# abdo-eldesokey/RAFT-NCUP

Hardware: AMD Instinct MI355X
Metric: train_image_pairs_per_sec (higher is better)
Workload: dtype bf16; 1 GPU; model=raft_nc_dbl, global_batch=3, refinement_iters=12, parallelism=dp1

## Files before the change

### csrc/bindings.cpp

```cpp

#include <torch/extension.h>

#include <vector>

#include <ATen/cuda/CUDAContext.h>
#include <c10/cuda/CUDAGuard.h>
#include <hip/hip_runtime.h>

void flowhip_bgemm_nt_launch(const void* A, const void* B, void* C,
                             float alpha, int batch, int M, int N, int K,
                             int out_bf16, hipStream_t stream);
void flowhip_corr_lookup_fwd_launch(const void* const* levels, const int* Hs,
                                    const int* Ws, const float* coords,
                                    void* out, int BP, int P,
                                    int L, int radius, int cl, int ldc,
                                    int is_bf16, hipStream_t stream);
void flowhip_corr_lookup_bwd_launch(const void* gout, const float* coords,
                                    void* const* glevels, const int* Hs,
                                    const int* Ws, int BP, int P,
                                    int L, int radius, int cl,
                                    int is_bf16, int acc,
                                    hipStream_t stream);
void flowhip_convex_up_fwd_launch(const float* flow, const float* mask,
                                  float* out, int N, int H, int W, int factor,
                                  hipStream_t stream);
void flowhip_convex_up_bwd_launch(const float* gout, const float* flow,
                                  const float* mask, float* gflow,
                                  float* gmask, int N, int H, int W,
                                  int factor, hipStream_t stream);
void flowhip_nconv_fwd_launch(const float* data, const float* conf,
                              const float* weight, const float* bias,
                              float* out, float* cout, int N, int Ci, int Co,
                              int H, int W, int K, hipStream_t stream);
void flowhip_nconv_bwd_data_launch(const float* dnomin, const float* ddenom,
                                   const float* data, const float* conf,
                                   const float* weight, float* ddata,
                                   float* dconf, int N, int Ci, int Co, int H,
                                   int W, int K, hipStream_t stream);
void flowhip_nconv_wrw_launch(const float* dnomin, const float* ddenom,
                              const float* data, const float* conf,
                              float* dweight, int N, int Ci, int Co, int H,
                              int W, int K, hipStream_t stream);
int flowhip_nconv_tiled_nblocks(int N, int H, int W, int Ci);
bool flowhip_nconv_fwd_tiled_launch(const float* data, const float* conf,
                                    const float* weight, const float* bias,
                                    float* out, float* cout, int N, int Ci,
                                    int Co, int H, int W, int K,
                                    hipStream_t stream);
bool flowhip_nconv_bwd_data_tiled_launch(
    const float* dnomin, const float* ddenom, const float* data,
    const float* conf, const float* weight, float* ddata, float* dconf, int N,
    int Ci, int Co, int H, int W, int K, hipStream_t stream);
bool flowhip_nconv_wrw_tiled_launch(const float* dnomin, const float* ddenom,
                                    const float* data, const float* conf,
                                    float* partials, float* dweight, int N,
                                    int Ci, int Co, int H, int W, int K,
                                    hipStream_t stream);
int flowhip_instnorm_partial_rows(int N, int C, long P);
void flowhip_conv_gemm_pack_launch(const float* w, void* wpk, long total,
                                   int O, int I, int KH, int KW, int cpad,
                                   int flip, hipStream_t stream);
void flowhip_transpose_cast_launch(const void* in, void* out, int B, int M,
                                   int N, int in_bf16, hipStream_t stream);
void flowhip_conf_pool_fwd_launch(const float* data, const float* conf,
                                  float* data_ds, float* conf_ds,
                                  unsigned char* code, long total, int H,
                                  int W, int OH, int OW, hipStream_t stream);
void flowhip_conf_pool_bwd_launch(const float* gdata_ds,
                                  const float* gconf_ds,
                                  const unsigned char* code, float* gdata,
                                  float* gconf, long total_in, int H, int W,
                                  int OH, int OW, hipStream_t stream);
void flowhip_conv_gemm_fwd_launch(const void* x, const void* x2,
                                  const void* wpk, const float* bias,
                                  void* out, void* out2, const void* zpage,
                                  long Mtot, int HH, int WW, int srcH,
                                  int srcW, int sH, int sW, int ld_x,
                                  int ld_x2, int C1, int Cin, int Cout,
                                  int cpad, int KH, int KW, int padH,
                                  int padW, int osplit, int act, int smode,
                                  hipStream_t stream);
void flowhip_conv_gemm_wrw_launch(const void* dy, const void* x,
                                  const void* x2, float* partials, float* dw,
                                  float* dbias,
                                  const void* zpage, long Mtot, int HH,
                                  int WW, int srcH, int srcW, int sH, int sW,
                                  int ld_x, int ld_x2, int C1,
                                  int Cin, int Cout, int cpad, int KH,
                                  int KW, int padH, int padW, int nchunk,
                                  hipStream_t stream);
void flowhip_instnorm_cl_fwd_launch(const void* x, void* y, float* mean,
                                    float* rstd, float* partials, int N,
                                    int C, long P, float eps, int is_bf16,
                                    hipStream_t stream);
void flowhip_instnorm_cl_bwd_launch(const void* x, const void* dy,
                                    const float* mean, const float* rstd,
                                    float* gmean, float* gxmean,
                                    float* partials, void* dx, int N, int C,
                                    long P, int is_bf16, hipStream_t stream);
void flowhip_zero_inject_fwd_launch(const float* inp, float* out, long total,
                                    int ih, int iw, int oh, int ow, int sH,
                                    int sW, hipStream_t stream);
void flowhip_zero_inject_bwd_launch(const float* gout, float* dinp,
                                    long total, int ih, int iw, int oh,
                                    int ow, int sH, int sW,
                                    hipStream_t stream);
void flowhip_gru_gate1_fwd_launch(const void* zr, const void* h, void* z,
                                  void* rh, long total, int C, long P,
                                  int is_bf16, int cl, hipStream_t stream);
void flowhip_gru_gate1_bwd_launch(const void* dz, const void* drh,
                                  const void* zr, const void* h, void* dzr,
                                  void* dh, long total, int C, long P,
                                  int is_bf16, int cl, hipStream_t stream);
void flowhip_gru_gate2_fwd_launch(const void* qp, const void* z,
                                  const void* h, void* hnew, long total,
                                  int is_bf16, hipStream_t stream);
void flowhip_gru_gate2_bwd_launch(const void* dhnew, const void* qp,
                                  const void* z, const void* h, void* dqp,
                                  void* dz, void* dh, long total, int is_bf16,
                                  hipStream_t stream);
void flowhip_seq_loss_fwd_launch(const float* const* preds, int n,
                                 const float* gt, const float* valid,
                                 float* partials, float* out, long npix,
                                 long plane, float max_flow, float gamma,
                                 long numel_full, hipStream_t stream);
void flowhip_seq_loss_bwd_launch(const float* const* preds, float* const* dst,
                                 int n, const float* gt, const float* valid,
                                 const float* gloss, long npix, long plane,
                                 float max_flow, float gamma, long numel_full,
                                 hipStream_t stream);
void flowhip_nconv_bwd_prep_launch(const float* gout, const float* gcout,
                                   const float* out, const float* cout,
                                   const float* wsum, const float* bias,
                                   float* dnomin, float* ddenom, long total,
                                   long plane, int Co, float eps,
                                   hipStream_t stream);
bool flowhip_col_sum2_launch(const void* g, const void* x, float* out,
                             long M, int C, int nchunk,
                             hipStream_t stream);
void flowhip_frozen_bn_apply_launch(const void* x, void* y, const float* s,
                                    const float* t, long M, int C,
                                    hipStream_t stream);
void flowhip_plane_dot_sum_launch(const float* x, const float* y, float* out,
                                  long P, int B, int C, hipStream_t stream);
bool flowhip_col_sum_launch(const void* dy, float* out,
                            long M, int C, int nchunk, hipStream_t stream);
void flowhip_up2x_cat_fwd_launch(const float* low, const float* skip,
                                 float* out, long total, int C1, int C2,
                                 int H, int W, hipStream_t stream);
void flowhip_area_up2x_fwd_launch(const float* in, float* out, long total,
                                  int H, int W, hipStream_t stream);
void flowhip_area_up2x_bwd_launch(const float* gout, float* gin,
                                  long total_in, int H, int W,
                                  hipStream_t stream);
bool flowhip_packernel_fwd_launch(const float* f, float* k, int B, int C,
                                  int H, int W, int K, int dil, int norm,
                                  hipStream_t stream);
bool flowhip_packernel_bwd_launch(const float* f, const float* k,
                                  const float* dk, float* df, int B, int C,
                                  int H, int W, int K, int dil, int norm,
                                  hipStream_t stream);
bool flowhip_pacconv_fwd_launch(const float* x, const float* kr,
                                const float* w, const float* bias, float* out,
                                int B, int Ci, int Co, int H, int W, int OH,
                                int OW, int pH, int pW, int K, int dil,
                                int shared, hipStream_t stream);
bool flowhip_pacconv_bwd_launch(const float* dy, const float* x,
                                const float* kr, const float* w, float* dx,
                                float* dk, float* partials, float* dw,
                                int nchunk, int B, int Ci, int Co, int H,
                                int W, int OH, int OW, int pH, int pW, int K,
                                int dil, int shared, hipStream_t stream);
void flowhip_pacpool_fwd_launch(const float* x, const float* kr, float* out,
// ... 670 lines not shown
  return wpk;
}

std::vector<torch::Tensor> conv_gemm_fwd2(
    torch::Tensor x, c10::optional<torch::Tensor> x2, torch::Tensor wpk,
    c10::optional<torch::Tensor> bias, int64_t Cout, int64_t KH, int64_t KW,
    int64_t osplit, int64_t act, int64_t sH, int64_t sW, int64_t smode,
    int64_t outH, int64_t outW) {
  int ld_x, ld_x2 = 0;
  cg_check_x(x, ld_x);
  TORCH_CHECK(wpk.is_cuda() && wpk.is_contiguous() &&
              wpk.scalar_type() == torch::kBFloat16 && wpk.dim() == 3);
  const int N = x.size(0), C1 = x.size(1), H = x.size(2), W = x.size(3);
  int Cin = C1;
  const void* x2p = nullptr;
  if (x2.has_value()) {
    int l2;
    cg_check_x(x2.value(), l2);
    TORCH_CHECK(x2->size(0) == N && x2->size(2) == H && x2->size(3) == W);
    TORCH_CHECK(C1 % 64 == 0, "conv_gemm cat2: first input must be a "
                "multiple of 64 channels");
    ld_x2 = l2;
    Cin = C1 + (int)x2->size(1);
    x2p = x2->data_ptr();
  }
  const int cpad = wpk.size(2);
  TORCH_CHECK(wpk.size(0) == KH * KW && wpk.size(1) == Cout);
  TORCH_CHECK(smode >= 0 && smode <= 2 && sH >= 1 && sW >= 1);
  int OH = H, OW = W;
  if (smode == 1) {
    OH = (int)((H + 2 * (KH / 2) - KH) / sH + 1);
    OW = (int)((W + 2 * (KW / 2) - KW) / sW + 1);
  } else if (smode == 2) {
    TORCH_CHECK(outH > 0 && outW > 0, "conv_gemm smode=2 needs outH/outW");
    OH = (int)outH; OW = (int)outW;
  }
  const long Mtot = (long)N * OH * OW;
  const float* bptr = nullptr;
  if (bias.has_value()) {
    TORCH_CHECK(bias->is_contiguous() &&
                bias->scalar_type() == torch::kFloat32 &&
                bias->numel() == Cout);
    bptr = bias->data_ptr<float>();
  }
  const c10::cuda::CUDAGuard guard(x.device());
  hipStream_t stream = at::cuda::getCurrentCUDAStream().stream();
  if (osplit <= 0 || osplit >= Cout) {
    auto out = torch::empty({(long)N, Cout, (long)OH, (long)OW}, x.options(),
                            torch::MemoryFormat::ChannelsLast);
    flowhip_conv_gemm_fwd_launch(x.data_ptr(), x2p, wpk.data_ptr(), bptr,
                                 out.data_ptr(), nullptr, cg_zero_page(),
                                 Mtot, OH, OW, H, W, (int)sH, (int)sW, ld_x,
                                 ld_x2, C1, Cin, (int)Cout,
                                 cpad, (int)KH, (int)KW, (int)KH / 2,
                                 (int)KW / 2, (int)Cout, (int)act,
                                 (int)smode, stream);
    return {out};
  }
  TORCH_CHECK(smode == 0, "conv_gemm: osplit only with smode 0");
  auto out = torch::empty({(long)N, osplit, (long)H, (long)W}, x.options(),
                          torch::MemoryFormat::ChannelsLast);
  auto out2 = torch::empty({(long)N, Cout - osplit, (long)H, (long)W},
                           x.options(), torch::MemoryFormat::ChannelsLast);
  flowhip_conv_gemm_fwd_launch(x.data_ptr(), x2p, wpk.data_ptr(), bptr,
                               out.data_ptr(), out2.data_ptr(),
                               cg_zero_page(), Mtot, H, W, H, W, 1, 1, ld_x,
                               ld_x2, C1,
                               Cin, (int)Cout, cpad, (int)KH, (int)KW,
                               (int)KH / 2, (int)KW / 2, (int)osplit,
                               (int)act, 0, stream);
  return {out, out2};
}

torch::Tensor conv_gemm_fwd(torch::Tensor x, torch::Tensor wpk,
                            c10::optional<torch::Tensor> bias, int64_t Cout,
                            int64_t KH, int64_t KW, int64_t act) {
  return conv_gemm_fwd2(x, c10::nullopt, wpk, bias, Cout, KH, KW, 0,
                        act, 1, 1, 0, 0, 0)[0];
}

std::vector<torch::Tensor> conv_gemm_wrw(torch::Tensor dy, torch::Tensor x,
                                         c10::optional<torch::Tensor> x2,
                                         int64_t KH, int64_t KW, int64_t sH,
                                         int64_t sW, bool want_bias) {
  int ld_x, ld_x2 = 0;
  cg_check_x(x, ld_x);
  TORCH_CHECK(dy.is_cuda() && dy.scalar_type() == torch::kBFloat16 &&
              dy.stride(1) == 1 && dy.stride(3) == dy.size(1),
              "conv_gemm_wrw: dy must be channels-last contiguous");
  const int N = x.size(0), C1 = x.size(1), H = x.size(2), W = x.size(3);
  const int OH = dy.size(2), OW = dy.size(3);
  TORCH_CHECK(dy.size(0) == N);
  int Cin = C1;
  const void* x2p = nullptr;
  if (x2.has_value()) {
    int l2;
    cg_check_x(x2.value(), l2);
    ld_x2 = l2;
    Cin = C1 + (int)x2->size(1);
    x2p = x2->data_ptr();
  }
  const int Cout = dy.size(1);
  const long Mtot = (long)N * OH * OW;
  const int cpad = (int)((Cin + 63) / 64) * 64;
  const int tiles_o = (Cout + 63) / 64;
  const int base_tiles = tiles_o * ((cpad + 63) / 64) * (int)(KH * KW);
  int nchunk = (512 + base_tiles - 1) / base_tiles;
  if (nchunk < 1) nchunk = 1;
  if (nchunk > 64) nchunk = 64;
  const long mtiles = (Mtot + 63) / 64;
  if (nchunk > mtiles) nchunk = (int)mtiles;
  auto partials = torch::empty(
      {(long)nchunk * KH * KW * tiles_o * 64 * cpad +
       (want_bias ? (long)nchunk * tiles_o * 64 : 0)},
      x.options().dtype(torch::kFloat32));
  auto dw = torch::empty({(long)Cout, (long)Cin, KH, KW},
                         x.options().dtype(torch::kFloat32));
  torch::Tensor dbias;
  if (want_bias)
    dbias = torch::empty({(long)Cout}, x.options().dtype(torch::kFloat32));
  const c10::cuda::CUDAGuard guard(x.device());
  hipStream_t stream = at::cuda::getCurrentCUDAStream().stream();
  flowhip_conv_gemm_wrw_launch(dy.data_ptr(), x.data_ptr(), x2p,
                               partials.data_ptr<float>(),
                               dw.data_ptr<float>(),
                               want_bias ? dbias.data_ptr<float>() : nullptr,
                               cg_zero_page(), Mtot,
                               OH, OW, H, W, (int)sH, (int)sW,
                               ld_x, ld_x2, C1, Cin, Cout, cpad, (int)KH,
                               (int)KW, (int)KH / 2, (int)KW / 2, nchunk,
                               stream);
  return {dw, dbias};
}

torch::Tensor col_sum_bf16(torch::Tensor dy) {
  TORCH_CHECK(dy.is_cuda() && dy.dim() == 4 &&
              dy.scalar_type() == torch::kBFloat16 && dy.stride(1) == 1 &&
              dy.stride(3) == dy.size(1));
  const int C = dy.size(1);
  const long M = dy.numel() / C;
  const int nchunk = (int)((M + 255) / 256);
  auto out = torch::zeros({(long)C}, dy.options().dtype(torch::kFloat32));
  const c10::cuda::CUDAGuard guard(dy.device());
  hipStream_t stream = at::cuda::getCurrentCUDAStream().stream();
  bool ok = flowhip_col_sum_launch(dy.data_ptr(),
                                   out.data_ptr<float>(), M, C, nchunk,
                                   stream);
  TORCH_CHECK(ok, "col_sum_bf16: C must be a multiple of 8");
  return out;
}

torch::Tensor plane_sum_nchw(torch::Tensor x, c10::optional<torch::Tensor> y) {
  TORCH_CHECK(x.is_cuda() && x.dim() == 4 && x.is_contiguous() &&
              x.scalar_type() == torch::kFloat32);
  const float* yp = nullptr;
  if (y.has_value()) {
    TORCH_CHECK(y->sizes() == x.sizes() && y->is_contiguous() &&
                y->scalar_type() == torch::kFloat32);
    yp = y->data_ptr<float>();
  }
  const int B = x.size(0), C = x.size(1);
  const long P = (long)x.size(2) * x.size(3);
  auto out = torch::zeros({(long)C}, x.options());
  const c10::cuda::CUDAGuard guard(x.device());
  hipStream_t stream = at::cuda::getCurrentCUDAStream().stream();
  flowhip_plane_dot_sum_launch(x.data_ptr<float>(), yp,
                               out.data_ptr<float>(), P, B, C, stream);
  return out;
}

torch::Tensor frozen_bn_apply(torch::Tensor x, torch::Tensor s,
                              c10::optional<torch::Tensor> t) {
  TORCH_CHECK(x.is_cuda() && x.dim() == 4 &&
              x.scalar_type() == torch::kBFloat16 && x.stride(1) == 1 &&
              x.stride(3) == x.size(1) && x.size(1) % 8 == 0);
  TORCH_CHECK(s.is_contiguous() && s.scalar_type() == torch::kFloat32 &&
              s.numel() == x.size(1));
  const float* tp = nullptr;
  if (t.has_value()) {
    TORCH_CHECK(t->is_contiguous() && t->scalar_type() == torch::kFloat32 &&
                t->numel() == x.size(1));
    tp = t->data_ptr<float>();
  }
  auto y = torch::empty_like(x);
  const c10::cuda::CUDAGuard guard(x.device());
  hipStream_t stream = at::cuda::getCurrentCUDAStream().stream();
  flowhip_frozen_bn_apply_launch(x.data_ptr(), y.data_ptr(),
                                 s.data_ptr<float>(), tp,
                                 x.numel() / x.size(1), (int)x.size(1),
                                 stream);
  return y;
}

torch::Tensor col_sum2_bf16(torch::Tensor g, torch::Tensor x) {
  TORCH_CHECK(g.is_cuda() && g.dim() == 4 &&
              g.scalar_type() == torch::kBFloat16 && g.stride(1) == 1 &&
              g.stride(3) == g.size(1));
  TORCH_CHECK(x.sizes() == g.sizes() && x.strides() == g.strides() &&
              x.scalar_type() == torch::kBFloat16);
  const int C = g.size(1);
  const long M = g.numel() / C;
  const int nchunk = (int)((M + 255) / 256);
  auto out = torch::zeros({2, (long)C}, g.options().dtype(torch::kFloat32));
  const c10::cuda::CUDAGuard guard(g.device());
  hipStream_t stream = at::cuda::getCurrentCUDAStream().stream();
  bool ok = flowhip_col_sum2_launch(g.data_ptr(), x.data_ptr(),
                                    out.data_ptr<float>(), M, C, nchunk,
                                    stream);
  TORCH_CHECK(ok, "col_sum2_bf16: C must be a multiple of 8");
  return out;
}

torch::Tensor up2x_cat_fwd(torch::Tensor low, torch::Tensor skip) {
  TORCH_CHECK(low.is_cuda() && low.is_contiguous() &&
// ... 148 lines not shown
                                       int64_t sH, int64_t sW, int64_t pH,
                                       int64_t pW, int64_t dil) {
  const int B = x.size(0), C = x.size(1), H = x.size(2), W = x.size(3);
  const int KCH = kr.size(1), OH = kr.size(3), OW = kr.size(4);
  auto dx = torch::zeros_like(x);
  auto dk = torch::empty_like(kr);
  const c10::cuda::CUDAGuard guard(x.device());
  hipStream_t stream = at::cuda::getCurrentCUDAStream().stream();
  flowhip_pacpool_bwd_launch(dy.contiguous().data_ptr<float>(),
                             x.data_ptr<float>(), kr.data_ptr<float>(),
                             dx.data_ptr<float>(), dk.data_ptr<float>(), B,
                             C, KCH, H, W, OH, OW, (int)K, (int)sH, (int)sW,
                             (int)pH, (int)pW, (int)dil, stream);
  return {dx, dk};
}

}

PYBIND11_MODULE(TORCH_EXTENSION_NAME, m) {
  m.doc() = "flowhip gfx950 HIP kernels";
  m.def("bgemm_nt", &bgemm_nt,
        "C[b] = alpha * A[b] (M,K) @ B[b] (N,K)^T, bf16 in / fp32|bf16 out",
        py::arg("a"), py::arg("b"), py::arg("alpha"),
        py::arg("out_bf16") = false);
  m.def("corr_lookup_fwd", &corr_lookup_fwd,
        "fused multi-level correlation window lookup (fp32/bf16 levels)");
  m.def("corr_lookup_bwd", &corr_lookup_bwd,
        "backward of corr_lookup_fwd (pyramid grads; accumulates into "
        "`prev` when the pyramid is iteration-chained)",
        py::arg("gout"), py::arg("coords"), py::arg("radius"),
        py::arg("level_shapes"), py::arg("channels_last"),
        py::arg("levels_bf16") = false,
        py::arg("prev") = py::none());
  m.def("corr_pyramid_fits", &corr_pyramid_fits,
        "does the fused pyramid-build kernel support this map size/dtype");
  m.def("packernel_fwd", &packernel_fwd, "PAC gaussian adapting kernel");
  m.def("packernel_bwd", &packernel_bwd, "backward of packernel_fwd");
  m.def("pacconv_fwd", &pacconv_fwd, "pixel-adaptive convolution forward");
  m.def("pacconv_bwd", &pacconv_bwd, "pixel-adaptive conv backward (dx,dk,dw)");
  m.def("pacpool_fwd", &pacpool_fwd, "pixel-adaptive pooling forward");
  m.def("pacpool_bwd", &pacpool_bwd,
        "pixel-adaptive pooling backward (dx via atomic scatter, dk)");
  m.def("corr_pyramid_fwd", &corr_pyramid_fwd,
        "fused avg-pool pyramid build (levels 1..n-1)");
  m.def("corr_pyramid_bwd", &corr_pyramid_bwd,
        "fused pyramid backward combine -> dcorr");
  m.def("convex_up_fwd", &convex_up_fwd, "fused convex-combination upsample");
  m.def("convex_up_bwd", &convex_up_bwd, "backward of convex_up_fwd");
  m.def("nconv_fwd", &nconv_fwd,
        "fused normalized convolution forward (out, cout)");
  m.def("plane_sum_nchw", &plane_sum_nchw,
        "out[c] = sum_{b,h,w} x (or x*y), NCHW fp32",
        py::arg("x"), py::arg("y") = py::none());
  m.def("frozen_bn_apply", &frozen_bn_apply,
        "y = bf16(fp32(x)*s + t) per channel, channels-last");
  m.def("col_sum2_bf16", &col_sum2_bf16,
        "(sum_m g, sum_m g*x) per channel in one pass (frozen-BN backward)");
  m.def("col_sum_bf16", &col_sum_bf16,
        "(N,C,H,W) channels-last bf16 -> (C) fp32 bias-grad column sum");
  m.def("up2x_cat_fwd", &up2x_cat_fwd,
        "fused nearest-2x upsample + channel concat");
  m.def("area_up2x_fwd", &area_up2x_fwd, "exact-2x area upsample");
  m.def("area_up2x_bwd", &area_up2x_bwd, "backward of area_up2x");
  m.def("conf_pool_fwd", &conf_pool_fwd,
        "confidence-based 2x pooling forward (data_ds, conf_ds, argmax code)");
  m.def("conf_pool_bwd", &conf_pool_bwd, "backward of conf_pool");
  m.def("transpose_cast_bf16", &transpose_cast_bf16,
        "(B,M,N) fp32 -> (B,N,M) bf16 tiled transpose");
  m.def("conv_gemm_pack", &conv_gemm_pack,
        "one-kernel conv weight packing (fwd or flipped-bwd layout)");
  m.def("conv_gemm_fwd", &conv_gemm_fwd,
        "implicit-GEMM NHWC bf16 conv forward (also bwd-data with flipped "
        "packed weights)");
  m.def("conv_gemm_fwd2", &conv_gemm_fwd2,
        "conv forward over a virtually-concatenated pair of inputs and/or "
        "with a split output (bwd-data of a cat input); smode 1 = strided "
        "direct conv, smode 2 = strided transposed conv (bwd-data)",
        py::arg("x"), py::arg("x2"), py::arg("wpk"), py::arg("bias"),
        py::arg("Cout"), py::arg("KH"), py::arg("KW"), py::arg("osplit"),
        py::arg("act"), py::arg("sH") = 1, py::arg("sW") = 1,
        py::arg("smode") = 0, py::arg("outH") = 0, py::arg("outW") = 0);
  m.def("conv_gemm_wrw", &conv_gemm_wrw,
        "implicit-GEMM conv weight gradient (split-M + reduce); returns "
        "[dw, dbias] — dbias undefined unless want_bias",
        py::arg("dy"), py::arg("x"), py::arg("x2"), py::arg("KH"),
        py::arg("KW"), py::arg("sH") = 1, py::arg("sW") = 1,
        py::arg("want_bias") = false);
  m.def("instnorm_cl_fwd", &instnorm_cl_fwd,
        "channels-last InstanceNorm2d forward (y, mean, rstd)");
  m.def("instnorm_cl_bwd", &instnorm_cl_bwd,
        "channels-last InstanceNorm2d backward");
  m.def("zero_inject_fwd", &zero_inject_fwd, "sparse injection scatter");
  m.def("zero_inject_bwd", &zero_inject_bwd, "backward gather of inject");
  m.def("gru_gate1_fwd", &gru_gate1_fwd, "fused GRU z/r gates + r*h");
  m.def("gru_gate1_bwd", &gru_gate1_bwd, "backward of gru_gate1");
  m.def("gru_gate2_fwd", &gru_gate2_fwd, "fused GRU tanh + lerp update");
  m.def("gru_gate2_bwd", &gru_gate2_bwd, "backward of gru_gate2");
  m.def("seq_loss_fwd", &seq_loss_fwd,
        "fused sequence loss forward -> [loss, epe, 1px, 3px, 5px]");
  m.def("seq_loss_bwd", &seq_loss_bwd,
        "fused sequence loss backward -> per-prediction grads");
  m.def("nconv_bwd_prep", &nconv_bwd_prep,
        "fused elementwise preamble of nconv backward (dnomin, ddenom)");
  m.def("nconv_bwd", &nconv_bwd,
        "fused normalized convolution backward (ddata, dconf, dweight)");
}
```

### csrc/conv_gemm.hip

```cpp

#include "common.h"

#define CG_BM 64
#define CG_BN 64
#define CG_BK 64
#define CG_THREADS 256

__device__ __forceinline__ unsigned cg_swz(unsigned row, unsigned slot) {
  return slot ^ ((row >> 1) & 7u);
}

template <int BM, int THREADS>
__device__ __forceinline__ void cg_coords(
    int wave, int lane, long m0, long Mtot, int HH, int WW,
    long* pn, int* pyy, int* pxx) {
  constexpr int PPT = BM * 8 / THREADS;
#pragma unroll
  for (int j = 0; j < PPT; ++j) {
    const int piece = wave * 64 + THREADS * j + lane;
    long m = m0 + (piece >> 3);
    if (m >= Mtot) m = Mtot - 1;
    pxx[j] = (int)(m % WW);
    pyy[j] = (int)((m / WW) % HH);
    pn[j] = m / ((long)WW * HH);
  }
}

template <int BM, int THREADS, int SMODE>
__device__ __forceinline__ void cg_stage_a(
    const __bf16* __restrict__ x, const __bf16* __restrict__ x2,
    const __bf16* __restrict__ zpage,
    char* lds_buf, int wave, int lane, const long* pn, const int* pyy,
    const int* pxx, int srcH, int srcW, int sH, int sW, int ld_x, int ld_x2,
    int C1, int Cin, int dy, int dx, int c0) {
  constexpr int PPT = BM * 8 / THREADS;
#pragma unroll
  for (int j = 0; j < PPT; ++j) {
    const int piece0 = wave * 64 + THREADS * j;
    const int piece = piece0 + lane;
    const int row = piece >> 3;
    const int slot = piece & 7;
    const int sslot = cg_swz(row, slot);
    const int xx = pxx[j];
    const int yy = pyy[j];
    const long n = pn[j];
    int sy, sx;
    bool ok;
    if (SMODE == 0) {
      sy = yy + dy; sx = xx + dx;
      ok = sy >= 0 && sy < srcH && sx >= 0 && sx < srcW;
    } else if (SMODE == 1) {
      sy = yy * sH + dy; sx = xx * sW + dx;
      ok = sy >= 0 && sy < srcH && sx >= 0 && sx < srcW;
    } else {
      const int ty = yy + dy, tx = xx + dx;
      sy = ty / sH; sx = tx / sW;
      ok = ty >= 0 && tx >= 0 && ty % sH == 0 && tx % sW == 0 &&
           sy < srcH && sx < srcW;
    }
    const int c = c0 + sslot * 8;
    const __bf16* src = zpage;
    if (ok && c < Cin) {
      if (x2 == nullptr || c < C1)
        src = x + (((long)n * srcH + sy) * srcW + sx) * ld_x + c;
      else
        src = x2 + (((long)n * srcH + sy) * srcW + sx) * ld_x2 + (c - C1);
    }
    __builtin_amdgcn_global_load_lds(
        (const __attribute__((address_space(1))) void*)src,
        (__attribute__((address_space(3))) void*)(lds_buf + piece0 * 16),
        16, 0, 0);
  }
}

template <int THREADS>
__device__ __forceinline__ void cg_stage_b(const __bf16* __restrict__ wsec,
                                           char* lds_buf, int wave, int lane,
                                           int n0, int Cout, int cpad,
                                           int c0) {
  constexpr int PPT = CG_BN * 8 / THREADS;
#pragma unroll
  for (int j = 0; j < PPT; ++j) {
    const int piece0 = wave * 64 + THREADS * j;
    if (piece0 >= CG_BN * 8) break;
// ... 384 lines not shown
    }
  const long total = (long)Cout * Cin * KYX;
  for (long idx = (long)blockIdx.x * CG_THREADS + threadIdx.x; idx < total;
       idx += (long)gridDim.x * CG_THREADS) {
    long t = idx;
    const int kyx = (int)(t % KYX); t /= KYX;
    const int c = (int)(t % Cin); t /= Cin;
    const int o = (int)t;
    float s = 0.f;
    for (int ch = 0; ch < nchunk; ++ch)
      s += partials[((((long)ch * KYX + kyx) * orows) + o) * cpad + c];
    dw[((long)o * Cin + c) * KYX + kyx] = s;
  }
}


template <int BM>
static void cg_fwd_dispatch(const __bf16* x, const __bf16* x2,
                            const __bf16* wpk, const float* bias, __bf16* out,
                            __bf16* out2, const __bf16* zpage, long Mtot,
                            int HH, int WW, int srcH, int srcW, int sH,
                            int sW, int ld_x, int ld_x2, int C1, int Cin,
                            int Cout, int cpad, int KH, int KW, int offH,
                            int offW, int osplit, int act, int smode,
                            hipStream_t stream) {
  const int tiles_m = (int)((Mtot + BM - 1) / BM);
  const int tiles_n = fh_cdiv(Cout, CG_BN);
  dim3 grid(tiles_m * tiles_n), block(BM == 64 ? 256 : 512);
#define CG_LAUNCH(A, S)                                                      \
  hipLaunchKernelGGL((conv_gemm_fwd_kernel<A, BM, S>), grid, block, 0,       \
                     stream, x, x2, wpk, bias, out, out2, zpage, Mtot, HH,   \
                     WW, srcH, srcW, sH, sW, ld_x, ld_x2, C1, Cin, Cout,     \
                     cpad, KH, KW, offH, offW, osplit, tiles_m)
  if (smode == 0) { if (act == 1) CG_LAUNCH(1, 0); else CG_LAUNCH(0, 0); }
  else if (smode == 1) { if (act == 1) CG_LAUNCH(1, 1); else CG_LAUNCH(0, 1); }
  else { if (act == 1) CG_LAUNCH(1, 2); else CG_LAUNCH(0, 2); }
#undef CG_LAUNCH
}

bool flowhip_conv_halo_fwd_launch(const void* x, const void* x2,
                                  const void* wpk, const float* bias,
                                  void* out, const void* zpage, int N,
                                  int H, int W, int ld_x, int ld_x2, int C1,
                                  int Cin, int Cout, int cpad, int ldo,
                                  int KH, int KW, int act,
                                  hipStream_t stream);

void flowhip_conv_gemm_fwd_launch(const void* x, const void* x2,
                                  const void* wpk, const float* bias,
                                  void* out, void* out2, const void* zpage,
                                  long Mtot, int HH, int WW, int srcH,
                                  int srcW, int sH, int sW, int ld_x,
                                  int ld_x2, int C1, int Cin, int Cout,
                                  int cpad, int KH, int KW, int padH,
                                  int padW, int osplit, int act, int smode,
                                  hipStream_t stream) {
  if (smode == 0 && out2 == nullptr && padH == KH / 2 && padW == KW / 2 &&
      ((KH == 3 && KW == 3) || (KH == 1 && KW == 5) ||
       (KH == 5 && KW == 1))) {
    const int N = (int)(Mtot / ((long)HH * WW));
    if (flowhip_conv_halo_fwd_launch(x, x2, wpk, bias, out, zpage, N, HH,
                                     WW, ld_x, ld_x2, C1, Cin, Cout, cpad,
                                     Cout, KH, KW, act, stream))
      return;
  }
  const int offH = smode == 2 ? padH - KH + 1 : -padH;
  const int offW = smode == 2 ? padW - KW + 1 : -padW;
  const long t128 = ((Mtot + 127) / 128) * fh_cdiv(Cout, CG_BN);
  if (t128 >= 320)
    cg_fwd_dispatch<128>((const __bf16*)x, (const __bf16*)x2,
                         (const __bf16*)wpk, bias, (__bf16*)out,
                         (__bf16*)out2, (const __bf16*)zpage, Mtot, HH, WW,
                         srcH, srcW, sH, sW, ld_x, ld_x2, C1, Cin, Cout,
                         cpad, KH, KW, offH, offW, osplit, act, smode,
                         stream);
  else
    cg_fwd_dispatch<64>((const __bf16*)x, (const __bf16*)x2,
                        (const __bf16*)wpk, bias, (__bf16*)out, (__bf16*)out2,
                        (const __bf16*)zpage, Mtot, HH, WW, srcH, srcW, sH,
                        sW, ld_x, ld_x2, C1, Cin, Cout, cpad, KH, KW, offH,
                        offW, osplit, act, smode, stream);
}

void flowhip_conv_gemm_wrw_launch(const void* dy, const void* x,
                                  const void* x2, float* partials, float* dw,
                                  float* dbias, const void* zpage, long Mtot,
                                  int HH,
                                  int WW, int srcH, int srcW, int sH, int sW,
                                  int ld_x, int ld_x2, int C1, int Cin,
                                  int Cout, int cpad, int KH, int KW,
                                  int padH, int padW, int nchunk,
                                  hipStream_t stream) {
  const int tiles_o = fh_cdiv(Cout, 64);
  const int tiles_c = fh_cdiv(cpad, 64);
  float* biasp = dbias
      ? partials + (long)nchunk * KH * KW * tiles_o * 64 * cpad
      : nullptr;
  dim3 block(CG_THREADS);
  dim3 grid(tiles_o * tiles_c, KH * KW, nchunk);
  hipLaunchKernelGGL(conv_gemm_wrw_kernel, grid, block, 0, stream,
                     (const __bf16*)dy, (const __bf16*)x,
                     (const __bf16*)x2, partials, biasp,
                     (const __bf16*)zpage,
                     Mtot, HH, WW, srcH, srcW, sH, sW, ld_x, ld_x2, C1,
                     Cin, Cout, cpad, KH, KW, padH, padW, tiles_o, tiles_c,
                     nchunk);
  const long total = (long)Cout * Cin * KH * KW;
  long rblocks = (total + CG_THREADS - 1) / CG_THREADS;
  if (rblocks > 4096) rblocks = 4096;
  hipLaunchKernelGGL(conv_gemm_wrw_reduce_kernel, dim3((int)rblocks), block,
                     0, stream, partials, dw, biasp, dbias, nchunk, KH * KW,
                     tiles_o * 64, cpad, Cout, Cin);
}

__global__ __launch_bounds__(256) void conv_gemm_pack_kernel(
    const float* __restrict__ w,
    __bf16* __restrict__ wpk,
    long total, int O, int I, int KH, int KW, int cpad, int flip) {
  const int KYX = KH * KW;
  for (long idx = (long)blockIdx.x * 256 + threadIdx.x; idx < total;
       idx += (long)gridDim.x * 256) {
    long t = idx;
    const int c = t % cpad; t /= cpad;
    const int r = t % (flip ? I : O); t /= (flip ? I : O);
    const int kyx = (int)t;
    float v = 0.f;
    if (!flip) {
      if (c < I) v = w[(((long)r * I + c) * KYX) + kyx];
    } else {
      const int ky = kyx / KW, kx = kyx - (kyx / KW) * KW;
      const int fk = (KH - 1 - ky) * KW + (KW - 1 - kx);
      if (c < O) v = w[(((long)c * I + r) * KYX) + fk];
    }
    wpk[idx] = (__bf16)v;
  }
}

void flowhip_conv_gemm_pack_launch(const float* w, void* wpk, long total,
                                   int O, int I, int KH, int KW, int cpad,
                                   int flip, hipStream_t stream) {
  long blocks = (total + 255) / 256;
  if (blocks > 4096) blocks = 4096;
  hipLaunchKernelGGL(conv_gemm_pack_kernel, dim3((int)blocks), dim3(256), 0,
                     stream, w, (__bf16*)wpk, total, O, I, KH, KW, cpad,
                     flip);
}
```

Before: 46.36 pairs/s.

## Add halo-staged weight-gradient conv kernel sharing input tile across all taps

Adds a new conv weight-gradient kernel for stride-1 same-padded 3x3, 1x5 and 5x1 convolutions. It stages a spatial tile of dy plus a haloed input tile into LDS once and computes every tap from that shared tile, instead of launching a separate per-tap GEMM that reloads the input. Staging is double-buffered with global_load_lds, reads use transpose LDS loads with swizzling, and a planner picks halo or the generic path automatically by tile count. The cost is a different split-M chunking scheme, higher register use (accumulators for every tap) and more code paths to keep correct.

```diff
diff --git a/csrc/bindings.cpp b/csrc/bindings.cpp
--- a/csrc/bindings.cpp
+++ b/csrc/bindings.cpp
@@ -80,7 +80,7 @@
                                   int cpad, int KH, int KW, int padH,
                                   int padW, int osplit, int act, int smode,
                                   hipStream_t stream);
-void flowhip_conv_gemm_wrw_launch(const void* dy, const void* x,
+bool flowhip_conv_gemm_wrw_launch(const void* dy, const void* x,
                                   const void* x2, float* partials, float* dw,
                                   float* dbias,
                                   const void* zpage, long Mtot, int HH,
@@ -88,7 +88,11 @@
                                   int ld_x, int ld_x2, int C1,
                                   int Cin, int Cout, int cpad, int KH,
                                   int KW, int padH, int padW, int nchunk,
-                                  hipStream_t stream);
+                                  int algo, hipStream_t stream);
+int flowhip_conv_gemm_wrw_plan(long Mtot, int HH, int WW, int srcH, int srcW,
+                               int sH, int sW, bool has_x2, int C1, int Cout,
+                               int cpad, int KH, int KW, int padH, int padW,
+                               int algo, int nchunk_req, int* nchunk_out);
 void flowhip_instnorm_cl_fwd_launch(const void* x, void* y, float* mean,
                                     float* rstd, float* partials, int N,
                                     int C, long P, float eps, int is_bf16,
@@ -925,7 +929,8 @@
 std::vector<torch::Tensor> conv_gemm_wrw(torch::Tensor dy, torch::Tensor x,
                                          c10::optional<torch::Tensor> x2,
                                          int64_t KH, int64_t KW, int64_t sH,
-                                         int64_t sW, bool want_bias) {
+                                         int64_t sW, bool want_bias,
+                                         int64_t algo, int64_t nchunk_req) {
   int ld_x, ld_x2 = 0;
   cg_check_x(x, ld_x);
   TORCH_CHECK(dy.is_cuda() && dy.scalar_type() == torch::kBFloat16 &&
@@ -947,12 +952,15 @@
   const long Mtot = (long)N * OH * OW;
   const int cpad = (int)((Cin + 63) / 64) * 64;
   const int tiles_o = (Cout + 63) / 64;
-  const int base_tiles = tiles_o * ((cpad + 63) / 64) * (int)(KH * KW);
-  int nchunk = (512 + base_tiles - 1) / base_tiles;
-  if (nchunk < 1) nchunk = 1;
-  if (nchunk > 64) nchunk = 64;
-  const long mtiles = (Mtot + 63) / 64;
-  if (nchunk > mtiles) nchunk = (int)mtiles;
+  TORCH_CHECK(algo >= -1 && algo <= 1, "conv_gemm_wrw: algo must be -1, 0, 1");
+  int nchunk = 1;
+  const int path = flowhip_conv_gemm_wrw_plan(
+      Mtot, OH, OW, H, W, (int)sH, (int)sW, x2p != nullptr, C1, Cout, cpad,
+      (int)KH, (int)KW, (int)KH / 2, (int)KW / 2, (int)algo, (int)nchunk_req,
+      &nchunk);
+  TORCH_CHECK(path >= 0,
+              "conv_gemm_wrw: algo=1 (halo) forced on a shape outside its "
+              "envelope (stride 1, same padding, 3x3 / 1x5 / 5x1)");
   auto partials = torch::empty(
       {(long)nchunk * KH * KW * tiles_o * 64 * cpad +
        (want_bias ? (long)nchunk * tiles_o * 64 : 0)},
@@ -964,7 +972,7 @@
     dbias = torch::empty({(long)Cout}, x.options().dtype(torch::kFloat32));
   const c10::cuda::CUDAGuard guard(x.device());
   hipStream_t stream = at::cuda::getCurrentCUDAStream().stream();
-  flowhip_conv_gemm_wrw_launch(dy.data_ptr(), x.data_ptr(), x2p,
+  const bool launched = flowhip_conv_gemm_wrw_launch(dy.data_ptr(), x.data_ptr(), x2p,
                                partials.data_ptr<float>(),
                                dw.data_ptr<float>(),
                                want_bias ? dbias.data_ptr<float>() : nullptr,
@@ -972,7 +980,9 @@
                                OH, OW, H, W, (int)sH, (int)sW,
                                ld_x, ld_x2, C1, Cin, Cout, cpad, (int)KH,
                                (int)KW, (int)KH / 2, (int)KW / 2, nchunk,
-                               stream);
+                               path, stream);
+  TORCH_CHECK(launched,
+              "conv_gemm_wrw: the halo kernel refused a planned shape");
   return {dw, dbias};
 }
 
@@ -1287,10 +1297,12 @@
         py::arg("smode") = 0, py::arg("outH") = 0, py::arg("outW") = 0);
   m.def("conv_gemm_wrw", &conv_gemm_wrw,
         "implicit-GEMM conv weight gradient (split-M + reduce); returns "
-        "[dw, dbias] — dbias undefined unless want_bias",
+        "[dw, dbias] — dbias undefined unless want_bias. algo: -1 auto, "
+        "0 generic per-tap kernel, 1 halo-staged kernel; nchunk: 0 auto",
         py::arg("dy"), py::arg("x"), py::arg("x2"), py::arg("KH"),
         py::arg("KW"), py::arg("sH") = 1, py::arg("sW") = 1,
-        py::arg("want_bias") = false);
+        py::arg("want_bias") = false, py::arg("algo") = -1,
+        py::arg("nchunk") = 0);
   m.def("instnorm_cl_fwd", &instnorm_cl_fwd,
         "channels-last InstanceNorm2d forward (y, mean, rstd)");
   m.def("instnorm_cl_bwd", &instnorm_cl_bwd,
diff --git a/csrc/conv_gemm.hip b/csrc/conv_gemm.hip
--- a/csrc/conv_gemm.hip
+++ b/csrc/conv_gemm.hip
@@ -1,5 +1,6 @@
 
 #include "common.h"
+#include "conv_wrw_halo_maps.h"
 
 #define CG_BM 64
 #define CG_BN 64
@@ -550,14 +551,59 @@
                         offW, osplit, act, smode, stream);
 }
 
-void flowhip_conv_gemm_wrw_launch(const void* dy, const void* x,
+bool flowhip_conv_wrw_halo_launch(const void* dy, const void* x,
+                                  const void* x2, float* partials,
+                                  float* biasp, const void* zpage, int N,
+                                  int H, int W, int ld_x, int ld_x2, int C1,
+                                  int Cin, int Cout, int cpad, int KH, int KW,
+                                  int nchunk, hipStream_t stream);
+
+int flowhip_conv_gemm_wrw_plan(long Mtot, int HH, int WW, int srcH, int srcW,
+                               int sH, int sW, bool has_x2, int C1, int Cout,
+                               int cpad, int KH, int KW, int padH, int padW,
+                               int algo, int nchunk_req, int* nchunk_out) {
+  const int tiles_o = fh_cdiv(Cout, 64);
+  const int tiles_c = fh_cdiv(cpad, 64);
+  const bool eligible =
+      sH == 1 && sW == 1 && srcH == HH && srcW == WW && padH == KH / 2 &&
+      padW == KW / 2 &&
+      ((KH == 3 && KW == 3) || (KH == 1 && KW == 5) ||
+       (KH == 5 && KW == 1)) &&
+      cpad % 64 == 0 && Cout % 8 == 0 && (!has_x2 || C1 % 64 == 0) &&
+      Mtot <= 0x7fffffffL;
+  if (algo == 1 && !eligible) return -1;
+  const long ptiles = eligible ? (Mtot / ((long)HH * WW)) *
+                                     fh_cdiv(HH, WH_TH) * fh_cdiv(WW, WH_TW)
+                               : 0;
+  const int tiles = tiles_o * tiles_c;
+  const bool wins = tiles >= 8 || (tiles >= 4 && ptiles >= 672);
+  const bool halo = eligible && (algo == 1 || (algo == -1 && wins));
+  if (halo) {
+    long n = nchunk_req > 0 ? nchunk_req : wh_nchunk(ptiles, tiles_o * tiles_c);
+    if (n > ptiles) n = ptiles;
+    if (n > 4096) n = 4096;
+    *nchunk_out = (int)n;
+    return 1;
+  }
+  const int base_tiles = tiles_o * tiles_c * KH * KW;
+  int nchunk = nchunk_req > 0 ? nchunk_req
+                              : (512 + base_tiles - 1) / base_tiles;
+  if (nchunk < 1) nchunk = 1;
+  if (nchunk > 64) nchunk = 64;
+  const long mtiles = (Mtot + 63) / 64;
+  if (nchunk > mtiles) nchunk = (int)mtiles;
+  *nchunk_out = nchunk;
+  return 0;
+}
+
+bool flowhip_conv_gemm_wrw_launch(const void* dy, const void* x,
                                   const void* x2, float* partials, float* dw,
                                   float* dbias, const void* zpage, long Mtot,
                                   int HH,
                                   int WW, int srcH, int srcW, int sH, int sW,
                                   int ld_x, int ld_x2, int C1, int Cin,
                                   int Cout, int cpad, int KH, int KW,
-                                  int padH, int padW, int nchunk,
+                                  int padH, int padW, int nchunk, int algo,
                                   hipStream_t stream) {
   const int tiles_o = fh_cdiv(Cout, 64);
   const int tiles_c = fh_cdiv(cpad, 64);
@@ -565,20 +611,29 @@
       ? partials + (long)nchunk * KH * KW * tiles_o * 64 * cpad
       : nullptr;
   dim3 block(CG_THREADS);
-  dim3 grid(tiles_o * tiles_c, KH * KW, nchunk);
-  hipLaunchKernelGGL(conv_gemm_wrw_kernel, grid, block, 0, stream,
-                     (const __bf16*)dy, (const __bf16*)x,
-                     (const __bf16*)x2, partials, biasp,
-                     (const __bf16*)zpage,
-                     Mtot, HH, WW, srcH, srcW, sH, sW, ld_x, ld_x2, C1,
-                     Cin, Cout, cpad, KH, KW, padH, padW, tiles_o, tiles_c,
-                     nchunk);
+  if (algo == 1) {
+    const int N = (int)(Mtot / ((long)HH * WW));
+    if (!flowhip_conv_wrw_halo_launch(dy, x, x2, partials, biasp, zpage, N,
+                                      HH, WW, ld_x, ld_x2, C1, Cin, Cout,
+                                      cpad, KH, KW, nchunk, stream))
+      return false;
+  } else {
+    dim3 grid(tiles_o * tiles_c, KH * KW, nchunk);
+    hipLaunchKernelGGL(conv_gemm_wrw_kernel, grid, block, 0, stream,
+                       (const __bf16*)dy, (const __bf16*)x,
+                       (const __bf16*)x2, partials, biasp,
+                       (const __bf16*)zpage,
+                       Mtot, HH, WW, srcH, srcW, sH, sW, ld_x, ld_x2, C1,
+                       Cin, Cout, cpad, KH, KW, padH, padW, tiles_o, tiles_c,
+                       nchunk);
+  }
   const long total = (long)Cout * Cin * KH * KW;
   long rblocks = (total + CG_THREADS - 1) / CG_THREADS;
   if (rblocks > 4096) rblocks = 4096;
   hipLaunchKernelGGL(conv_gemm_wrw_reduce_kernel, dim3((int)rblocks), block,
                      0, stream, partials, dw, biasp, dbias, nchunk, KH * KW,
                      tiles_o * 64, cpad, Cout, Cin);
+  return true;
 }
 
 __global__ __launch_bounds__(256) void conv_gemm_pack_kernel(
diff --git a/csrc/conv_wrw_halo.hip b/csrc/conv_wrw_halo.hip
--- /dev/null
+++ b/csrc/conv_wrw_halo.hip
@@ -0,0 +1,222 @@
+
+#include "common.h"
+#include "conv_wrw_halo_maps.h"
+
+typedef __attribute__((ext_vector_type(4))) short wh_s16x4;
+typedef __attribute__((ext_vector_type(8))) short wh_s16x8;
+
+#define WH_TR(dst, addr, imm)                                   \
+  asm volatile("ds_read_b64_tr_b16 %0, %1 offset:%2"            \
+               : "=v"(dst)                                      \
+               : "v"(addr), "n"(imm)                            \
+               : "memory")
+
+template <int KYX>
+struct WhFrag {
+  wh_s16x4 alo[4], ahi[4], blo[KYX], bhi[KYX];
+};
+
+template <int KH, int KW>
+__global__ __launch_bounds__(WH_THREADS) void conv_wrw_halo_kernel(
+    const __bf16* __restrict__ dy,
+    const __bf16* __restrict__ x,
+    const __bf16* __restrict__ x2,
+    float* __restrict__ partials,
+    float* __restrict__ biasp,
+    const __bf16* __restrict__ zpage,
+    int N, int H, int W, int ld_x, int ld_x2, int C1, int Cin, int Cout,
+    int cpad, int tiles_o, int ntx, int nty, int nchunk) {
+  constexpr int KYX = KH * KW;
+  constexpr int LW = (WH_TW + KW - 1 + 7) / 8 * 8;
+  constexpr int XP = (WH_TH + KH - 1) * LW * 8;
+  constexpr int BUF = WH_DY_BYTES + XP * 16;
+  __shared__ __attribute__((aligned(16))) char lds[2 * BUF];
+
+  const int wave = threadIdx.x >> 6;
+  const int lane = threadIdx.x & 63;
+  const int to = blockIdx.x % tiles_o;
+  const int tc = blockIdx.x / tiles_o;
+  const int chunk = blockIdx.y;
+  const int o0 = to * 64, c0 = tc * 64;
+
+  const long ptiles = (long)N * nty * ntx;
+  const int t0 = (int)((ptiles * chunk) / nchunk);
+  const int t1 = (int)((ptiles * (chunk + 1)) / nchunk);
+
+  f32x4 acc[KYX][4];
+#pragma unroll
+  for (int t = 0; t < KYX; ++t)
+#pragma unroll
+    for (int i = 0; i < 4; ++i) acc[t][i] = {0.f, 0.f, 0.f, 0.f};
+
+  const bool do_bias = biasp != nullptr && tc == 0 && wave == 0;
+  float bacc[4] = {0.f, 0.f, 0.f, 0.f};
+
+  const WhLane L = wh_lane_init(lane, wave);
+  const unsigned lds0 =
+      (unsigned)(unsigned long)((__attribute__((address_space(3))) char*)lds);
+  const WhStage S = wh_stage_init(threadIdx.x, KW);
+  const bool from2 = x2 != nullptr && c0 >= C1;
+  const __bf16* const xs = from2 ? x2 : x;
+  const int xld = from2 ? ld_x2 : ld_x;
+  const int cbase = from2 ? c0 - C1 : c0;
+
+  auto stage = [&](int t, char* dimg, char* ximg) {
+    const int txi = t % ntx;
+    const int r = t / ntx;
+    const int tyi = r % nty;
+    const int n = r / nty;
+    const int x0 = txi * WH_TW, y0 = tyi * WH_TH;
+
+#pragma unroll
+    for (int j = 0; j < WH_DY_PIECES / WH_THREADS; ++j) {
+      const int piece0 = wave * 64 + WH_THREADS * j;
+      const long off = wh_dy_src_thr(S, j, n, y0, x0, H, W, Cout, o0);
+      const __bf16* src = off < 0 ? zpage : dy + off;
+      __builtin_amdgcn_global_load_lds(
+          (const __attribute__((address_space(1))) void*)src,
+          (__attribute__((address_space(3))) void*)(dimg + piece0 * 16), 16,
+          0, 0);
+    }
+    int px = S.px0, py = S.py0;
+#pragma unroll 1
+    for (int piece0 = wave * 64; piece0 < XP; piece0 += WH_THREADS) {
+      const long off = wh_x_src_thr(S, px, py, n, y0, x0, H, W, KH, KW, xld,
+                                    cbase, c0, Cin);
+      const __bf16* src = off < 0 ? zpage : xs + off;
+      __builtin_amdgcn_global_load_lds(
+          (const __attribute__((address_space(1))) void*)src,
+          (__attribute__((address_space(3))) void*)(ximg + piece0 * 16), 16,
+          0, 0);
+      wh_x_step(px, py, KW);
+    }
+  };
+
+  if (t0 < t1) stage(t0, lds, lds + WH_DY_BYTES);
+  int cur = 0;
+  for (int t = t0; t < t1; ++t) {
+    asm volatile("s_waitcnt vmcnt(0)" ::: "memory");
+    __syncthreads();
+    if (t + 1 < t1)
+      stage(t + 1, lds + (cur ^ 1) * BUF, lds + (cur ^ 1) * BUF + WH_DY_BYTES);
+
+    unsigned da[4], xa[KW];
+#pragma unroll
+    for (int i = 0; i < 4; ++i) da[i] = lds0 + (unsigned)cur * BUF + L.dy[i];
+#pragma unroll
+    for (int kx = 0; kx < KW; ++kx)
+      xa[kx] = lds0 + (unsigned)cur * BUF + WH_DY_BYTES + L.x[kx];
+
+    WhFrag<KYX> F[2];
+    auto issue = [&](WhFrag<KYX>& f, int ks) {
+#pragma unroll
+      for (int i = 0; i < 4; ++i) {
+        WH_TR(f.alo[i], da[i], wh_dy_kstep(ks) + wh_dy_imm(0));
+        WH_TR(f.ahi[i], da[i], wh_dy_kstep(ks) + wh_dy_imm(1));
+      }
+#pragma unroll
+      for (int tap = 0; tap < KYX; ++tap) {
+        const int ky = tap / KW, kx = tap % KW;
+        WH_TR(f.blo[tap], xa[kx], wh_x_kstep(ks, KW) + wh_x_imm(0, ky, KW));
+        WH_TR(f.bhi[tap], xa[kx], wh_x_kstep(ks, KW) + wh_x_imm(1, ky, KW));
+      }
+    };
+    auto landed = [&](WhFrag<KYX>& f) {
+      asm volatile("s_waitcnt lgkmcnt(0)" ::: "memory");
+#pragma unroll
+      for (int i = 0; i < 4; ++i)
+        asm volatile("" : "+v"(f.alo[i]), "+v"(f.ahi[i]));
+#pragma unroll
+      for (int tap = 0; tap < KYX; ++tap)
+        asm volatile("" : "+v"(f.blo[tap]), "+v"(f.bhi[tap]));
+    };
+    issue(F[0], 0);
+    landed(F[0]);
+#pragma unroll
+    for (int ks = 0; ks < WH_TH; ++ks) {
+      WhFrag<KYX>& f = F[ks & 1];
+      if (ks + 1 < WH_TH) issue(F[(ks + 1) & 1], ks + 1);
+      __builtin_amdgcn_sched_barrier(0);
+      bf16x8 af[4];
+#pragma unroll
+      for (int i = 0; i < 4; ++i)
+        af[i] = __builtin_bit_cast(
+            bf16x8, __builtin_shufflevector(f.alo[i], f.ahi[i], 0, 1, 2, 3, 4,
+                                            5, 6, 7));
+      if (do_bias) {
+#pragma unroll
+        for (int i = 0; i < 4; ++i)
+#pragma unroll
+          for (int e = 0; e < 8; ++e) bacc[i] += (float)af[i][e];
+      }
+#pragma unroll
+      for (int tap = 0; tap < KYX; ++tap) {
+        const bf16x8 bfr = __builtin_bit_cast(
+            bf16x8, __builtin_shufflevector(f.blo[tap], f.bhi[tap], 0, 1, 2,
+                                            3, 4, 5, 6, 7));
+#pragma unroll
+        for (int i = 0; i < 4; ++i)
+          acc[tap][i] = __builtin_amdgcn_mfma_f32_16x16x32_bf16(
+              af[i], bfr, acc[tap][i], 0, 0, 0);
+      }
+      __builtin_amdgcn_sched_barrier(0);
+      if (ks + 1 < WH_TH) landed(F[(ks + 1) & 1]);
+    }
+    cur ^= 1;
+  }
+
+  const int orows = tiles_o * 64;
+  const int fcol = lane & 15;
+  const int frow0 = (lane >> 4) * 4;
+#pragma unroll
+  for (int tap = 0; tap < KYX; ++tap) {
+    float* pbase = partials + (((long)chunk * KYX + tap) * orows) * cpad;
+#pragma unroll
+    for (int i = 0; i < 4; ++i)
+#pragma unroll
+      for (int rr = 0; rr < 4; ++rr) {
+        const int o = o0 + i * 16 + frow0 + rr;
+        const int c = c0 + wave * 16 + fcol;
+        pbase[(long)o * cpad + c] = acc[tap][i][rr];
+      }
+  }
+
+  if (do_bias) {
+#pragma unroll
+    for (int i = 0; i < 4; ++i) {
+      float s = bacc[i];
+      s += __shfl_xor(s, 16, 64);
+      s += __shfl_xor(s, 32, 64);
+      if (lane < 16) biasp[(long)chunk * orows + o0 + i * 16 + lane] = s;
+    }
+  }
+}
+
+bool flowhip_conv_wrw_halo_launch(const void* dy, const void* x,
+                                  const void* x2, float* partials,
+                                  float* biasp, const void* zpage, int N,
+                                  int H, int W, int ld_x, int ld_x2, int C1,
+                                  int Cin, int Cout, int cpad, int KH, int KW,
+                                  int nchunk, hipStream_t stream) {
+  if (cpad % 64 != 0 || Cout % 8 != 0) return false;
+  if (x2 != nullptr && C1 % 64 != 0) return false;
+  const int tiles_o = fh_cdiv(Cout, 64), tiles_c = cpad / 64;
+  const int ntx = fh_cdiv(W, WH_TW), nty = fh_cdiv(H, WH_TH);
+  const long ptiles = (long)N * nty * ntx;
+  if (nchunk < 1 || nchunk > ptiles || nchunk > 65535 ||
+      (long)N * H * W > 0x7fffffffL)
+    return false;
+  dim3 grid(tiles_o * tiles_c, nchunk), block(WH_THREADS);
+#define WH_LAUNCH(KHH, KWW)                                                  \
+  if (KH == KHH && KW == KWW) {                                              \
+    hipLaunchKernelGGL((conv_wrw_halo_kernel<KHH, KWW>), grid, block, 0,     \
+                       stream, (const __bf16*)dy, (const __bf16*)x,          \
+                       (const __bf16*)x2, partials, biasp,                   \
+                       (const __bf16*)zpage, N, H, W, ld_x, ld_x2, C1, Cin,  \
+                       Cout, cpad, tiles_o, ntx, nty, nchunk);               \
+    return true;                                                             \
+  }
+  WH_LAUNCH(3, 3) WH_LAUNCH(1, 5) WH_LAUNCH(5, 1)
+#undef WH_LAUNCH
+  return false;
+}
diff --git a/csrc/conv_wrw_halo_maps.h b/csrc/conv_wrw_halo_maps.h
--- /dev/null
+++ b/csrc/conv_wrw_halo_maps.h
@@ -0,0 +1,165 @@
+#pragma once
+
+#ifndef __HIPCC__
+#ifndef __host__
+#define __host__
+#endif
+#ifndef __device__
+#define __device__
+#endif
+#endif
+
+#define WH_TH 4
+#define WH_TW 32
+#define WH_THREADS 256
+#define WH_DY_PIECES (WH_TH * WH_TW * 8)
+#define WH_DY_BYTES (WH_DY_PIECES * 16)
+
+__host__ __device__ inline int wh_lw(int KW) {
+  return (WH_TW + KW - 1 + 7) / 8 * 8;
+}
+__host__ __device__ inline int wh_lh(int KH) { return WH_TH + KH - 1; }
+__host__ __device__ inline int wh_x_pieces(int KH, int KW) {
+  return wh_lh(KH) * wh_lw(KW) * 8;
+}
+__host__ __device__ inline int wh_lds_bytes(int KH, int KW) {
+  return WH_DY_BYTES + wh_x_pieces(KH, KW) * 16;
+}
+
+__host__ __device__ inline unsigned wh_swz(unsigned pix) {
+  return (pix >> 1) & 3u;
+}
+__host__ __device__ inline int wh_piece_chan(int piece) {
+  const unsigned pix = (unsigned)piece >> 3, slot = (unsigned)piece & 7u;
+  return (int)((((slot >> 1) ^ wh_swz(pix)) << 4) + ((slot & 1u) << 3));
+}
+
+__host__ __device__ inline long wh_dy_src(int piece, int n, int y0, int x0,
+                                          int H, int W, int Cout, int o0) {
+  const int pix = piece >> 3;
+  const int gy = y0 + pix / WH_TW, gx = x0 + pix % WH_TW;
+  const int o = o0 + wh_piece_chan(piece);
+  if (gy >= H || gx >= W || o >= Cout) return -1;
+  return (((long)n * H + gy) * W + gx) * Cout + o;
+}
+
+__host__ __device__ inline long wh_x_src(int piece, int n, int y0, int x0,
+                                         int H, int W, int KH, int KW,
+                                         int ld_x, int ld_x2, int C1,
+                                         int Cin, bool has_x2, int c0,
+                                         int* which) {
+  const int LW = wh_lw(KW);
+  const int pix = piece >> 3;
+  const int py = pix / LW, px = pix - py * LW;
+  const int gy = y0 + py - KH / 2, gx = x0 + px - KW / 2;
+  const int c = c0 + wh_piece_chan(piece);
+  *which = 0;
+  if (px >= WH_TW + KW - 1 || gy < 0 || gy >= H || gx < 0 || gx >= W ||
+      c >= Cin)
+    return 0;
+  const long p = ((long)n * H + gy) * W + gx;
+  if (!has_x2 || c < C1) {
+    *which = 1;
+    return p * ld_x + c;
+  }
+  *which = 2;
+  return p * ld_x2 + (c - C1);
+}
+
+struct WhStage {
+  int tx;
+  int chan;
+  int px0, py0;
+};
+__host__ __device__ inline WhStage wh_stage_init(int tid, int KW) {
+  WhStage S;
+  S.tx = tid >> 3;
+  S.chan = wh_piece_chan(tid);
+  S.py0 = (tid >> 3) / wh_lw(KW);
+  S.px0 = (tid >> 3) - S.py0 * wh_lw(KW);
+  return S;
+}
+__host__ __device__ inline long wh_dy_src_thr(const WhStage& S, int j, int n,
+                                              int y0, int x0, int H, int W,
+                                              int Cout, int o0) {
+  const int gy = y0 + j, gx = x0 + S.tx, o = o0 + S.chan;
+  if (gy >= H || gx >= W || o >= Cout) return -1;
+  return (long)(((n * H + gy) * W) + gx) * Cout + o;
+}
+__host__ __device__ inline void wh_x_step(int& px, int& py, int KW) {
+  px += 32;
+  if (px >= wh_lw(KW)) {
+    px -= wh_lw(KW);
+    ++py;
+  }
+}
+__host__ __device__ inline long wh_x_src_thr(const WhStage& S, int px, int py,
+                                             int n, int y0, int x0, int H,
+                                             int W, int KH, int KW, int ld,
+                                             int cbase, int c0, int Cin) {
+  const int gy = y0 + py - KH / 2, gx = x0 + px - KW / 2;
+  if (px >= WH_TW + KW - 1 || gy < 0 || gy >= H || gx < 0 || gx >= W ||
+      c0 + S.chan >= Cin)
+    return -1;
+  return (long)(((n * H + gy) * W) + gx) * ld + (cbase + S.chan);
+}
+
+__host__ __device__ inline int wh_tr_tx(int lane, int h) {
+  return h * 16 + (lane >> 4) * 4 + ((lane >> 2) & 3);
+}
+__host__ __device__ inline unsigned wh_tr_addr(unsigned pix, int cb,
+                                               int lane) {
+  return pix * 128u + (((unsigned)cb ^ wh_swz(pix)) << 5) +
+         ((unsigned)lane & 3u) * 8u;
+}
+__host__ __device__ inline unsigned wh_dy_pix(int ks, int tx) {
+  return (unsigned)(ks * WH_TW + tx);
+}
+__host__ __device__ inline unsigned wh_x_pix(int ks, int tx, int ky, int kx,
+                                             int KW) {
+  return (unsigned)((ks + ky) * wh_lw(KW) + tx + kx);
+}
+
+struct WhLane {
+  unsigned dy[4];
+  unsigned x[5];
+};
+__host__ __device__ inline WhLane wh_lane_init(int lane, int cbx) {
+  WhLane L;
+  const unsigned tx = (unsigned)wh_tr_tx(lane, 0);
+  const unsigned base = tx * 128u + ((unsigned)lane & 3u) * 8u;
+  for (int i = 0; i < 4; ++i)
+    L.dy[i] = base + (((unsigned)i ^ ((tx >> 1) & 3u)) << 5);
+  for (unsigned kx = 0; kx < 5; ++kx)
+    L.x[kx] = base + kx * 128u +
+              (((unsigned)cbx ^ (((kx >> 1) + ((tx + (kx & 1u)) >> 1)) & 3u))
+               << 5);
+  return L;
+}
+__host__ __device__ constexpr unsigned wh_dy_imm(int h) {
+  return (unsigned)h * 16u * 128u;
+}
+__host__ __device__ constexpr unsigned wh_x_imm(int h, int ky, int KW) {
+  return (unsigned)(ky * ((WH_TW + KW - 1 + 7) / 8 * 8) + h * 16) * 128u;
+}
+__host__ __device__ constexpr unsigned wh_dy_kstep(int ks) {
+  return (unsigned)ks * WH_TW * 128u;
+}
+__host__ __device__ constexpr unsigned wh_x_kstep(int ks, int KW) {
+  return (unsigned)ks * ((WH_TW + KW - 1 + 7) / 8 * 8) * 128u;
+}
+__host__ __device__ inline unsigned wh_dy_addr(const WhLane& L, int ks, int h,
+                                               int i) {
+  return L.dy[i] + wh_dy_kstep(ks) + wh_dy_imm(h);
+}
+__host__ __device__ inline unsigned wh_x_addr(const WhLane& L, int ks, int h,
+                                              int ky, int kx, int KW) {
+  return L.x[kx] + wh_x_kstep(ks, KW) + wh_x_imm(h, ky, KW);
+}
+
+__host__ __device__ inline int wh_nchunk(long ptiles, int tiles) {
+  long n = (192 + tiles / 2) / tiles;
+  if (n > ptiles) n = ptiles;
+  if (n < 1) n = 1;
+  return (int)n;
+}
```

Result: faster. 47.14 pairs/s, median of 6 (+1.7%).
